# tan9zj/xnrs

Measured on AMD Instinct MI355X. Metric: impressions/sec (encode+score) on MIND-shaped batches, higher is better.
Workload: dtype f32; 1 GPU; NRMS full user+news encode + 5-candidate dot scoring (BASELINE configs[2]; token shape of config/mind_small_NRMS.yml); batch_impressions_per_gpu=512, history=50, candidates=5, d_backbone=768, n_heads=16, emb_dim=256, parallelism=impressions sharded by user over 1 GPU(s), no data-path collective

## Files before the change

include/xnrs_hip.h:

```cpp
#ifndef XNRS_HIP_H
#define XNRS_HIP_H

#include <stddef.h>
#include <stdint.h>

#ifdef __cplusplus
extern "C" {
#endif

#define XNRS_ABI_VERSION 6

#define XNRS_OK 0
#define XNRS_EINVAL (-1)
#define XNRS_EHEADS (-2)
#define XNRS_EWORKSPACE (-3)
#define XNRS_EUNSUPPORTED (-4)

#define XNRS_ACT_NONE 0
#define XNRS_ACT_RELU 1
#define XNRS_ACT_TANH 2

#define XNRS_POOL_ADDITIVE 0
#define XNRS_POOL_MEAN 1

// ... 185 lines not shown
                          uint64_t seed, const uint64_t *seed_dev, void *stream);

int32_t xnrs_gather_rows_bf16(const uint16_t *table, const int32_t *ids, float *out, int64_t n, int64_t row_elems,
                              void *stream);
int32_t xnrs_dropout_rows_bf16(const uint16_t *table, const int32_t *ids, float *out, int64_t n, int64_t row_elems,
                               float p, uint64_t seed, const uint64_t *seed_dev, void *stream);

int32_t xnrs_assemble_train_batch(const int64_t *sess, int64_t B, const int64_t *hist_off, const int32_t *hist_val,
                                  const int64_t *pos_off, const int32_t *pos_val, const int64_t *neg_off,
                                  const int32_t *neg_val, int32_t l_hist, int32_t n_neg, int32_t pad_row, uint64_t seed,
                                  int32_t *hist_rows, int32_t *cand_rows, void *stream);
int32_t xnrs_assemble_eval_batch(const int64_t *sess, int64_t B, const int64_t *hist_off, const int32_t *hist_val,
                                 const int64_t *pos_off, const int32_t *pos_val, const int64_t *neg_off,
                                 const int32_t *neg_val, int32_t l_hist, int32_t pad_row, const int64_t *cand_off,
                                 int32_t *hist_rows, int32_t *cand_rows, int32_t *cand_sess, float *targets, void *stream);
int32_t xnrs_score_csr(const float *vecs, const int32_t *cand_rows, const int32_t *cand_sess, const float *u, float *r,
                       int64_t n_cand, int32_t E, int32_t relu, void *stream);
int32_t xnrs_rank_metrics(const float *scores, const float *targets, const int64_t *cand_off, float *out, int64_t B,
                          void *stream);

size_t xnrs_infonce_saved_bytes(int64_t B, int32_t E);
int32_t xnrs_infonce_fwd(const float *emb, const int64_t *labels, int64_t B, int32_t E, float temperature, float *loss,
                         void *saved, size_t saved_bytes, void *stream);
int32_t xnrs_infonce_bwd(const int64_t *labels, int64_t B, int32_t E, float temperature, const void *saved,
                         size_t saved_bytes, const float *gout, float *demb, void *stream);

#define XNRS_PROFILE_STAGES 10
int32_t xnrs_profile_enable(uint32_t stage_mask);
int32_t xnrs_profile_read(double *ms, int64_t *launches, double *flops);

int32_t xnrs_qkv_launch_count(int32_t reset);
int32_t xnrs_qkv_one_launch_map(int64_t block, int64_t live_tiles, int64_t live_rows, int32_t kv_row_tiles,
                                int32_t kv_col_tiles, int64_t q_rows, int32_t q_tile_rows, int32_t q_col_tiles,
                                int32_t *section, int32_t *index);

int32_t xnrs_train_fold_enabled(void);

#define XNRS_STATUS_NONBINARY_MASK 1
#define XNRS_STATUS_ROW_RANGE 2
#define XNRS_STATUS_QUERY_RANGE 4
int32_t xnrs_set_status_word(int32_t *device_word);
const char *xnrs_status_string(int32_t word);

#define XNRS_GEMM_F32 0
#define XNRS_GEMM_BF16X3 1
#define XNRS_GEMM_BF16X2 2
int32_t xnrs_set_gemm_mode(int32_t mode);
int32_t xnrs_get_gemm_mode(void);

int32_t xnrs_reload_knobs(void);

size_t xnrs_bilinear_scoring_saved_bytes(int64_t B, int32_t E, int32_t normalize);
int32_t xnrs_bilinear_scoring_fwd(const float *u, const float *c, const float *w, const float *bias, float *s, int64_t B,
                                  int32_t N, int32_t E, int32_t normalize, void *saved, size_t saved_bytes, void *stream);
size_t xnrs_bilinear_scoring_bwd_workspace_bytes(int64_t B, int32_t E, int32_t normalize);
int32_t xnrs_bilinear_scoring_bwd(const float *u, const float *c, const float *w, const void *saved, size_t saved_bytes,
                                  const float *ds, float *du, float *dc, float *dw, float *dbias, int64_t B, int32_t N,
                                  int32_t E, int32_t normalize, void *ws, size_t ws_bytes, void *stream);
size_t xnrs_mlp_scoring_saved_bytes(int64_t B, int32_t N, int32_t H);
int32_t xnrs_mlp_scoring_fwd(const float *u, const float *c, const float *w1, const float *b1, const float *w2,
                             const float *b2, float *s, int64_t B, int32_t N, int32_t E, int32_t H, void *saved,
                             size_t saved_bytes, void *stream);
size_t xnrs_mlp_scoring_bwd_workspace_bytes(int64_t B, int32_t N, int32_t H);
int32_t xnrs_mlp_scoring_bwd(const float *u, const float *c, const float *w1, const float *w2, const void *saved,
                             size_t saved_bytes, const float *ds, float *du, float *dc, float *dw1, float *db1, float *dw2,
                             float *db2, int64_t B, int32_t N, int32_t E, int32_t H, void *ws, size_t ws_bytes,
// ... 93 lines not shown
```

xnrs_amd/csrc/api.hip:

```cpp
#include <mutex>
#include <vector>

#include "host.h"

using namespace xnrs;

namespace xnrs {
uint32_t g_prof_mask = 0;
}
namespace {
std::vector<ProfRec> g_prof;
std::mutex g_prof_mu;
constexpr size_t PROF_MAX = 1 << 16;
}

bool xnrs::prof_begin(ProfRec* r, hipStream_t stream) {
  if (hipEventCreate(&r->beg) != hipSuccess || hipEventCreate(&r->end) != hipSuccess) return false;
  (void)hipEventRecord(r->beg, stream);
  return true;
}

void xnrs::prof_end(const ProfRec& r, hipStream_t stream) {
  (void)hipEventRecord(r.end, stream);
  std::lock_guard<std::mutex> lk(g_prof_mu);
// ... 56 lines not shown
  const int prev = xnrs::gemm_mode();
  xnrs::set_gemm_mode(mode);
  return prev;
}

int32_t xnrs_get_gemm_mode(void) { return xnrs::gemm_mode(); }

int32_t xnrs_train_fold_enabled(void) { return fold_wanted(knobs().fold_train) ? 1 : 0; }

int32_t xnrs_reload_knobs(void) {
  xnrs::reload_knobs();
  return XNRS_OK;
}

int32_t xnrs_qkv_launch_count(int32_t reset) {
  const int64_t n = xnrs::qkv_launches_read(reset != 0);
  return n > 0x7fffffffLL ? 0x7fffffff : (int32_t)n;
}

int32_t xnrs_qkv_one_launch_map(int64_t block, int64_t live_tiles, int64_t live_rows, int32_t kv_row_tiles, int32_t kv_col_tiles,
                                int64_t q_rows, int32_t q_tile_rows, int32_t q_col_tiles, int32_t* section, int32_t* index) {
  if (kv_row_tiles < 0 || kv_col_tiles < 1 || q_rows < 0 || q_tile_rows < 1 || q_col_tiles < 1) return XNRS_EINVAL;
  const int64_t grid = xnrs::qkv_one_launch_grid(kv_row_tiles, kv_col_tiles, q_rows, q_tile_rows, q_col_tiles);
  if (grid > 0x7fffffffLL) return XNRS_EINVAL;
  if (section && index) {
    const xnrs::QkvOneLaunchWork w =
        xnrs::qkv_one_launch_map(block, live_tiles, live_rows, kv_row_tiles, kv_col_tiles, q_rows, q_tile_rows, q_col_tiles);
    *section = w.section;
    *index = w.index;
  }
  return (int32_t)grid;
}

int32_t xnrs_profile_enable(uint32_t stage_mask) {
  std::lock_guard<std::mutex> lk(g_prof_mu);
  for (auto& r : g_prof) {
    (void)hipEventDestroy(r.beg);
    (void)hipEventDestroy(r.end);
  }
  g_prof.clear();
  g_prof_mask = stage_mask;
  return XNRS_OK;
}

int32_t xnrs_profile_read(double* ms, int64_t* launches, double* flops) {
  if (!ms || !launches || !flops) return XNRS_EINVAL;
  for (int i = 0; i < XNRS_PROFILE_STAGES; ++i) {
    ms[i] = 0.0;
    launches[i] = 0;
    flops[i] = 0.0;
  }
  int32_t rc = XNRS_OK;
  std::lock_guard<std::mutex> lk(g_prof_mu);
  for (auto& r : g_prof) {
    float t = 0.f;
    hipError_t e = hipEventSynchronize(r.end);
    if (e == hipSuccess) e = hipEventElapsedTime(&t, r.beg, r.end);
    if (e != hipSuccess) rc = (int32_t)e;
    else {
      ms[r.stage] += t;
      launches[r.stage] += 1;
      flops[r.stage] += r.flops;
    }
    (void)hipEventDestroy(r.beg);
    (void)hipEventDestroy(r.end);
  }
// ... 6 lines not shown
```

xnrs_amd/csrc/encoder_fwd.hip:

```cpp
#include <vector>

#include "host.h"

using namespace xnrs;

namespace xnrs {

Plan make_plan(int64_t n_seq, int L, int D, int A, int E, bool att, bool additive, bool head, bool pooled, int64_t chunk,
               bool train, int n_heads, bool widen) {
  Plan p{};
  if (train) chunk = n_seq > 0 ? n_seq : 1;
  if (chunk <= 0) chunk = 65536 / L;
  if (chunk > n_seq) chunk = n_seq;
  if (chunk < 1) chunk = 1;
  p.chunk = chunk;
  const size_t rows = (size_t)chunk * L;
  Carver c;
  p.off_qkv = c.take_if(att, rows * 3 * (size_t)D * F32);
  p.off_o = c.take_if(att, rows * (size_t)D * F32);
  p.off_y = c.take_if(att && pooled, rows * (size_t)D * F32);
  p.off_t = c.take_if(pooled && additive, rows * (size_t)A * F32);
  p.off_p = c.take_if(pooled && head, (size_t)n_seq * D * F32);
  p.off_h = c.take_if(pooled && head, (size_t)n_seq * E * F32);
  p.off_stats = c.take_if(train && att, (size_t)chunk * n_heads * L * 2 * F32);
// ... 369 lines not shown
    probe.mask = m;
    probe.skip_dead = 1;
    lt_qkv = mha_core_skips_dead(probe);
  }
  const bool lt_fc1 = lt && additive && rowdot;
  const int64_t lt_cap = live_tiles_cap(p.chunk, L, LIVE_TILE_BM);
  const int64_t* lt_n = at<int64_t>(w, p.off_lt_n);
  const int32_t* lt_tiles = at<int32_t>(w, p.off_lt_tiles);
  const bool lr = lt && knobs().gemm_live_rows && p.off_lr_cnt != 0 && L <= 64 && n_seq * (int64_t)L <= 0x7fffffffLL &&
                  n_seq * (int64_t)L >= knobs().gemm_live_rows_min_rows;
  const bool lr_qkv = lr && lt_qkv && !direct, lr_fc1 = lr && lt_fc1;
  const int32_t *lr_loc = at<int32_t>(w, p.off_lr_loc), *lr_src = at<int32_t>(w, p.off_lr_src);
  const int64_t* lr_cnt = at<int64_t>(w, p.off_lr_cnt);
  constexpr float LR_FILL = 0.3f;
  if (lr_qkv || lr_fc1)
    XNRS_TRY(launch_dense_row_lists(m, ids, n_seq, p.chunk, L, LIVE_TILE_BM, at<int32_t>(w, p.off_lr_loc), at<int32_t>(w, p.off_lr_src),
                                    at<int64_t>(w, p.off_lr_cnt), at<uint8_t>(w, p.off_lt_alive), at<int64_t>(w, p.off_lt_n),
                                    at<int32_t>(w, p.off_lt_tiles), stream));
  else if (lt_qkv || lt_fc1)
    XNRS_TRY(launch_live_tiles(m, ids, n_seq, p.chunk, L, LIVE_TILE_BM, at<uint8_t>(w, p.off_lt_alive), at<int64_t>(w, p.off_lt_n),
                               at<int32_t>(w, p.off_lt_tiles), stream));
  std::vector<int64_t> lt_host, lr_host;
  if ((lt_qkv && prof_on(0)) || (lt_fc1 && prof_on(3))) {
    lt_host.resize((size_t)((n_seq + p.chunk - 1) / p.chunk));
    if (hipStreamSynchronize(stream) != hipSuccess ||
        hipMemcpy(lt_host.data(), lt_n, lt_host.size() * sizeof(int64_t), hipMemcpyDeviceToHost) != hipSuccess)
      lt_host.clear();
    if (lr_qkv || lr_fc1) {
      lr_host.resize(3 * lt_host.size());
      if (lt_host.empty() || hipMemcpy(lr_host.data(), lr_cnt, lr_host.size() * sizeof(int64_t), hipMemcpyDeviceToHost) != hipSuccess)
        lr_host.clear();
    }
  }
  for (int64_t c0 = 0; !fused && !afused && c0 < n_seq; c0 += p.chunk) {
    const int64_t nc = (n_seq - c0 < p.chunk) ? (n_seq - c0) : p.chunk;
    const int64_t rows = nc * L;
    const int64_t* ltn = lt_n + c0 / p.chunk;
    const int32_t* ltl = lt_tiles + (c0 / p.chunk) * lt_cap;
    const double lt_rows = (double)LIVE_TILE_BM *
                           (double)(lt_host.empty() ? (rows + LIVE_TILE_BM - 1) / LIVE_TILE_BM : lt_host[(size_t)(c0 / p.chunk)]);
    const int32_t* lrl = lr_loc + (c0 / p.chunk) * p.chunk * L;
    const int32_t* lrs = lr_src + (c0 / p.chunk) * p.chunk * L;
    const int64_t* lrn = lr_cnt + 3 * (c0 / p.chunk);
    const double lr_rows = lr_host.empty() ? (double)rows : (double)lr_host[(size_t)(3 * (c0 / p.chunk))];
    const int32_t* cids = ids ? ids + c0 : nullptr;
    const float* cx = ids ? x : x + c0 * (int64_t)L * D;
    const float* cm = m ? (ids ? m : m + c0 * (int64_t)L) : nullptr;
    const int32_t* xids = cids;
    if (x16) {
      cx = direct ? nullptr : x32;
      xids = direct ? cids : nullptr;
      if (!direct) XNRS_TRY(widen_pass(c0, nc, false));
    }

    const float* seq = cx;
    const int32_t* seq_ids = xids;
    if (att) {
      const int64_t ld3 = 3 * (int64_t)D;
      if (qkv_given) {
      } else if (live) {
        const double nl = (double)prof_count(0, cnt, 0, n_live, stream), nkv = (double)prof_count(0, cnt, 1, n_kv, stream);
        ProfScope ps(0, 2.0 * (kvl ? nkv : rows) * 2.0 * D * D + 2.0 * nl * (double)D * D, stream);
        GemmArgs g = qkv_projection(cx, {xids, L}, att, 1, qkv + D, ld3, rows, D, pqkv);
        if (kvl) {
          XNRS_TRY(launch_zero_dead_qkv(qkv, cm, cids, nc, L, D, stream));
          g.gather_ids = kvx;
          g.gather_S = 1;
          g.c_scatter = 1;
          g.c_scatter_ids = kv_rows;
          g.M = n_kv;
          g.m_dev = cnt ? cnt + 1 : nullptr;
          g.m_fill_hint = 0.6f;
          if (n_kv > 0) XNRS_TRY(launch_gemm_f32(g, stream));
        } else {
          XNRS_TRY(launch_gemm_f32(g, stream));
          XNRS_TRY(launch_zero_cols(qkv, ld3, D, rows, stream));
        }
        if (n_live > 0) {
          GemmArgs q = gemm_linear(cx, {lvx, 1}, D, att->wq, att->bq, qkv, ld3, n_live, D, D, XNRS_ACT_NONE, pqkv[0]);
          q.c_scatter = 1;
          q.c_scatter_ids = live_rows;
          q.m_dev = cnt;
          q.m_fill_hint = 0.4f;
          XNRS_TRY(launch_gemm_f32(q, stream));
        }
      } else if (lr_qkv) {
        ProfScope ps(0, 2.0 * lt_rows * 2.0 * D * D + 2.0 * lr_rows * (double)D * D, stream);
        GemmArgs g = qkv_projection(cx, {xids, L}, att, 1, qkv + D, ld3, rows, D, pqkv);
        g.live_n = ltn;
        g.live_tiles = ltl;
        GemmArgs q = gemm_linear(cx, {xids ? lrs : lrl, 1}, D, att->wq, att->bq, qkv, ld3, rows, D, D);
        q.c_scatter = 1;
        q.c_scatter_ids = lrl;
        q.m_dev = lrn;
        q.m_fill_hint = LR_FILL;
        if (gemm_qkv_one_launch_ok(g, q)) {
          XNRS_TRY(launch_gemm_qkv_one(g, q, stream));
          qkv_launches_add(1);
        } else {
          XNRS_TRY(launch_gemm_f32(g, stream));
          XNRS_TRY(launch_gemm_f32(q, stream));
          qkv_launches_add(2);
        }
      } else {
        GemmArgs g = qkv_projection(cx, {xids, L}, att, 0, qkv, ld3, rows, D, pqkv);
        if (lt_qkv) {
          g.live_n = ltn;
          g.live_tiles = ltl;
        }
        ProfScope ps(0, 2.0 * (lt_qkv ? lt_rows : (double)rows) * 3.0 * D * D, stream);
        if (direct) XNRS_TRY(launch_gemm_a16(g, x16, stream));
        else XNRS_TRY(launch_gemm_f32(g, stream));
      }

      MhaCoreArgs ma = mha_core_args(qkv + D, ld3, att, o, nc, L, D);
      ma.q = qkv;
      ma.mask = cm;
      ma.mask_gather_ids = cids;
      ma.dropout_p = att->dropout_p;
      ma.seed = att->seed + (uint64_t)c0 * (uint64_t)att->n_heads * 0x9E3779B97F4A7C15ull;
      ma.seed_dev = att->seed_dev;
      ma.stats = stats;
      ma.skip_dead = (live || (pooled && cm && knobs().mha_skip_masked)) ? 1 : 0;
      if (lt_qkv && !mha_core_skips_dead(ma)) return XNRS_EUNSUPPORTED;
      {
        ProfScope ps(1, 4.0 * rows * (double)L * D, stream);
        XNRS_TRY(launch_mha_core(ma, stream));
      }

      float* dst = pooled ? yb : y + c0 * (int64_t)L * D;
      if (fold) {
        dst = o;
      } else if (live) {
        ProfScope ps(2, 2.0 * (double)prof_count(2, cnt, 0, n_live, stream) * (double)D * D, stream);
        XNRS_TRY(hipMemsetAsync(dst, 0, (size_t)rows * D * sizeof(float), stream));
// ... 3 lines not shown
          og.m_dev = cnt;
          og.m_fill_hint = 0.4f;
          XNRS_TRY(launch_gemm_f32(og, stream));
        }
      } else {
        ProfScope ps(2, 2.0 * rows * (double)D * D, stream);
        XNRS_TRY(launch_gemm_f32(gemm_linear(o, {}, D, att->wo, att->bo, dst, D, rows, D, D, XNRS_ACT_NONE, po), stream));
      }
      seq = dst;
      seq_ids = nullptr;
    }
    if (!pooled) continue;

    float* pooled_dst = (head ? pb : y) + c0 * (int64_t)D;
    float* hm_dst = hm ? hm + c0 : nullptr;
    if (additive) {
      if (live) {
        ProfScope ps(3, 2.0 * (double)prof_count(3, cnt, 0, n_live, stream) * (double)D * A, stream);
        XNRS_TRY(hipMemsetAsync(t, 0, (size_t)rows * A * sizeof(float), stream));
        if (n_live > 0) {
          GemmArgs fg = fc1_product(seq, {att ? live_rows : lvx, 1}, fc1, t, n_live, D, A, false, pool, p1);
          fg.c_scatter = 1;
          fg.c_scatter_ids = live_rows;
          fg.m_dev = cnt;
          fg.m_fill_hint = 0.4f;
          XNRS_TRY(launch_gemm_f32(fg, stream));
        }
      } else if (lr_fc1) {
        GemmArgs fg = fc1_product(seq, {seq_ids ? lrs : lrl, 1}, fc1, t, rows, D, A, true, pool, p1);
        fg.c_scatter = 1;
        fg.c_scatter_ids = lrl;
        fg.m_dev = lrn;
        fg.m_fill_hint = LR_FILL;
        ProfScope ps(3, 2.0 * lr_rows * (double)D * A, stream);
        XNRS_TRY(launch_gemm_f32(fg, stream));
      } else {
        GemmArgs fg = fc1_product(seq, {seq_ids, L}, fc1, t, rows, D, A, rowdot, pool, p1);
        if (lt_fc1) {
          fg.live_n = ltn;
          fg.live_tiles = ltl;
        }
        ProfScope ps(3, 2.0 * (lt_fc1 ? lt_rows : (double)rows) * (double)D * A, stream);
        XNRS_TRY(launch_gemm_f32(fg, stream));
      }
      AdditivePoolArgs pa = additive_pool_args(t, rowdot, pool, seq, nc, L, D, A);
      pa.skip_dead = lt_fc1 ? 1 : 0;
      pa.skip_masked = lr_fc1 ? 1 : 0;
      pa.mask = cm;
      pa.mask_gather_ids = cids;
      pa.x_gather_ids = seq_ids;
      pa.y = fold ? pob + c0 * (int64_t)D : pooled_dst;
      pa.asum_out = fold ? asum + c0 : nullptr;
      pa.a_out = a_save ? a_save : (a_out ? a_out + c0 * (int64_t)L : nullptr);
      pa.hm_out = cm ? hm_dst : nullptr;
      {
        ProfScope ps(4, 2.0 * rows * (double)(A + D), stream);
        XNRS_TRY(launch_additive_pool(pa, stream));
      }
      if (a_save && a_out)
        XNRS_TRY(hipMemcpyAsync(a_out, a_save, (size_t)rows * sizeof(float), hipMemcpyDeviceToDevice, stream));
    } else {
      MeanPoolArgs mp{};
      mp.x = seq;
      mp.ldx = D;
      mp.mask = cm;
      mp.mask_gather_ids = cids;
      mp.x_gather_ids = seq_ids;
      mp.y = pooled_dst;
      mp.hm_out = hm_dst;
      mp.n_seq = nc;
      mp.N = L;
      mp.D = D;
      {
        ProfScope ps(4, 2.0 * rows * (double)D, stream);
        XNRS_TRY(launch_mean_pool(mp, stream));
      }
    }
  }
  return pooled_tail(fold, pob, asum, att, pooled ? head : nullptr, pb, hb, y, n_seq, D, E, po, train, stream);
}

namespace {

struct UnpadPlan {
  size_t off_kv, off_q, off_o, off_y, off_t, off_p, off_h;
  FoldRegions fold;
  size_t total;
};
UnpadPlan make_unpad_plan(int64_t n_news, int64_t n_valid, int S, int D, int A, int E, bool att, bool head) {
  UnpadPlan p{};
  Carver c;
  const size_t nv = (size_t)(n_valid > 0 ? n_valid : 1);
  p.off_kv = c.take_if(att, (size_t)n_news * S * 2 * D * F32);
  p.off_q = c.take_if(att, nv * D * F32);
  p.off_o = c.take_if(att, nv * D * F32);
  p.off_y = c.take_if(att, nv * D * F32);
  p.off_t = c.take(nv * A * F32);
  p.off_p = c.take_if(head, (size_t)n_news * D * F32);
  p.off_h = c.take_if(head, (size_t)n_news * E * F32);
  p.fold = carve_fold(c, att, n_news, D, A);
  p.total = c.total();
  return p;
}

struct CompactPlan {
  int64_t chunk;
  size_t off_kv, off_q, off_o, off_t, off_roff, off_live, off_kvs, off_kvb, off_cnt, off_p, off_h;
  FoldRegions fold;
  size_t total;
};
CompactPlan make_compact_plan(int64_t n_news, int S, int D, int A, int E, bool att, bool head, int64_t chunk) {
// ... 339 lines not shown
```

xnrs_amd/csrc/gemm_f32.hip:

```cpp
#include <atomic>
#include <cstdlib>
#include <type_traits>

#include "kernels.h"

namespace xnrs {

constexpr int KALIGN = 32;

__device__ __attribute__((aligned(16))) float g_zero_line[4] = {0.f, 0.f, 0.f, 0.f};

typedef unsigned u32x4 __attribute__((ext_vector_type(4)));
constexpr unsigned BUF_OOB = 0x40000000u;

template <int TM, int TN, bool A_COL, bool B_KN, bool VEC, int PIPE, int BK, bool BUF = false, int MINW = 2, bool GATH = false,
          int KG = 2, bool RDOT = false, bool MDEV = false, bool LIVE = false>
__global__ __launch_bounds__(256, MINW) void gemm_f32_kernel(const GemmArgs a, int m_tiles, int n_tiles_seg, int gn) {
#define XNRS_GEMM_BID blockIdx.x
#define XNRS_GEMM_NWG gridDim.x
#define XNRS_GEMM_LDS_TILES(A, B)                            \
  __shared__ __attribute__((aligned(16))) float A[NBUF][A_SZ]; \
  __shared__ __attribute__((aligned(16))) float B[NBUF][B_SZ];
#include "gemm_f32_body.h"
#undef XNRS_GEMM_BID
// ... 9 lines not shown
template <int TM, int TN, bool A_COL, bool B_KN, bool VEC, int PIPE, int BK, bool BUF = false, int MINW = 2, bool GATH = false,
          int KG = 2, bool RDOT = false, bool MDEV = false, bool LIVE = false>
__device__ __forceinline__ void gemm_f32_body(const GemmArgs& a, int m_tiles, const int n_tiles_seg, const int gn, const int bid_in,
                                              const int nwg_in, float* As0, float* Bs0) {
  static_assert(!A_COL && !B_KN, "forward layout (the LDS tile sizes of gemm_f32_lds_floats)");
#define XNRS_GEMM_BID bid_in
#define XNRS_GEMM_NWG nwg_in
#define XNRS_GEMM_LDS_TILES(A, B)                                                                                   \
  static_assert(NBUF * A_SZ == gemm_f32_lds_floats<TM, BK>() && NBUF * B_SZ == gemm_f32_lds_floats<TN, BK>(), "LDS"); \
  float(*const A)[A_SZ] = reinterpret_cast<float(*)[A_SZ]>(As0);                                                    \
  float(*const B)[B_SZ] = reinterpret_cast<float(*)[B_SZ]>(Bs0);
#include "gemm_f32_body.h"
#undef XNRS_GEMM_BID
#undef XNRS_GEMM_NWG
#undef XNRS_GEMM_LDS_TILES
}

__global__ __launch_bounds__(256, 4) void gemm_qkv_one_launch_kernel(const GemmArgs kv, const GemmArgs q, int kv_m_tiles,
                                                                     int kv_n_tiles_seg, int kv_gn, int q_m_tiles, int q_n_tiles,
                                                                     int q_gn) {
  __shared__ __attribute__((aligned(16))) float As[gemm_f32_lds_floats<2, 16>()];
  __shared__ __attribute__((aligned(16))) float Bs[gemm_f32_lds_floats<2, 16>()];
  static_assert(sizeof(As) + sizeof(Bs) <= 32768, "four workgroups per CU");
  const int64_t ln = __builtin_amdgcn_readfirstlane((int)load_dev_scalar(kv.live_n));
  const int64_t md0 = load_dev_scalar(q.m_dev);
  const int64_t md = ((int64_t)__builtin_amdgcn_readfirstlane((int)(md0 >> 32)) << 32) | (uint32_t)__builtin_amdgcn_readfirstlane((int)md0);
  const QkvOneLaunchWork w = qkv_one_launch_map((int64_t)blockIdx.x, ln, md, kv_m_tiles, kv_n_tiles_seg * kv.nseg, q.M, 128, q_n_tiles);
  if (w.section < 0) return;
  if (w.section == 0)
    gemm_f32_body<2, 2, false, false, true, 5, 16, true, 4, false, 2, false, false, true>(kv, kv_m_tiles, kv_n_tiles_seg, kv_gn, w.index, 0,
                                                                                        As, Bs);
  else
    gemm_f32_body<2, 1, false, false, true, 5, 16, true, 4, true, 2, false, true, false>(q, q_m_tiles, q_n_tiles, q_gn, w.index, 0, As, Bs);
}

__global__ __launch_bounds__(256) void transpose_kernel(const float* W, float* Wt, int rows, int cols) {
  __shared__ float tile[32][33];
  const int tx = threadIdx.x & 31, ty = threadIdx.x >> 5;
  const int c0 = blockIdx.x * 32, r0 = blockIdx.y * 32;
#pragma unroll
  for (int i = 0; i < 4; ++i) {
    const int r = r0 + ty + 8 * i, c = c0 + tx;
    if (r < rows && c < cols) tile[ty + 8 * i][tx] = W[(int64_t)r * cols + c];
  }
  __syncthreads();
#pragma unroll
  for (int i = 0; i < 4; ++i) {
    const int c = c0 + ty + 8 * i, r = r0 + tx;
    if (r < rows && c < cols) Wt[(int64_t)c * rows + r] = tile[tx][ty + 8 * i];
  }
}

__global__ __launch_bounds__(256) void zero_cols_kernel(float* p, int64_t ld, int w4, int64_t n4) {
  const int64_t i = (int64_t)blockIdx.x * 256 + threadIdx.x;
  if (i >= n4) return;
  const int64_t r = i / w4;
  const int c = (int)(i - r * w4);
  __builtin_nontemporal_store(f32x4{0.f, 0.f, 0.f, 0.f}, reinterpret_cast<f32x4*>(p + r * ld) + c);
}

hipError_t launch_zero_cols(float* p, int64_t ld, int width, int64_t rows, hipStream_t stream) {
  if (rows <= 0 || width <= 0) return hipSuccess;
  if (width % 4 != 0 || ld % 4 != 0 || (reinterpret_cast<uintptr_t>(p) & 15) != 0)
    return hipMemset2DAsync(p, (size_t)ld * sizeof(float), 0, (size_t)width * sizeof(float), (size_t)rows, stream);
  const int64_t n4 = rows * (width / 4);
  hipLaunchKernelGGL(zero_cols_kernel, dim3((unsigned)((n4 + 255) / 256)), dim3(256), 0, stream, p, ld, width / 4, n4);
// ... 206 lines not shown
  return (int)ns;
}

static Knobs read_knobs() {
  Knobs k;
  auto num = [](const char* name, long long dflt) {
    const char* e = getenv(name);
    return (e && *e) ? atoll(e) : dflt;
  };
  k.gemm_pipe = (int)num("XNRS_GEMM_PIPE", 6);
  k.gemm_bk = num("XNRS_GEMM_BK", 32) == 16 ? 16 : 32;
  k.gemm_buf = num("XNRS_GEMM_BUF", 1) != 0;
  k.gemm_group = num("XNRS_GEMM_GROUP", -1);
  k.gemm_tile = (int)num("XNRS_GEMM_TILE", -1);
  k.split_min_tiles = num("XNRS_GEMM_SPLIT_MIN_TILES", 512);
  k.mha_lds = (int)num("XNRS_MHA_LDS", -1);
  k.mha_headwave = num("XNRS_MHA_HEADWAVE", 1) != 0;
  k.mha_pair = num("XNRS_MHA_PAIR", 1) != 0;
  k.mha_bwd_fused = num("XNRS_MHA_BWD_FUSED", 1) != 0;
  k.gemm_dw = (int)num("XNRS_GEMM_DW", 2);
  k.gemm_dw_tile = (int)num("XNRS_GEMM_DW_TILE", 256);
  k.fold_out = (int)num("XNRS_FOLD_OUT", 1);
  k.fc1_rowdot = num("XNRS_FC1_ROWDOT", 1) != 0;
  k.fold_train = (int)num("XNRS_FOLD_TRAIN", 1);
  k.news_fused = (int)num("XNRS_NEWS_FUSED", 1);
  k.news_fused_npw = (int)num("XNRS_NEWS_FUSED_NPW", 0);
  k.fast_tanh = num("XNRS_FAST_TANH", 1) != 0;
  k.additive_fused = (int)num("XNRS_ADDITIVE_FUSED", 1);
  k.af_fbuf = num("XNRS_AF_FBUF", 1) == 2 ? 2 : 1;
  k.mha_skip_masked = num("XNRS_MHA_SKIP_MASKED", 1) != 0;
  {
    k.gemm_qkv_one_launch = num("XNRS_GEMM_QKV_ONE_LAUNCH", 1) != 0;
  }
  k.gemm_live_tiles = num("XNRS_GEMM_LIVE_TILES", 1) != 0;
  k.gemm_live_tiles_min_rows = num("XNRS_GEMM_LIVE_TILES_MIN_ROWS", 16384);
  k.gemm_live_rows = num("XNRS_GEMM_LIVE_ROWS", 1) != 0;
  k.gemm_live_rows_min_rows = num("XNRS_GEMM_LIVE_ROWS_MIN_ROWS", 16384);
  k.bwd_side_stream = num("XNRS_BWD_SIDE_STREAM", 1) != 0;
  k.bwd_side_min_rows = num("XNRS_BWD_SIDE_MIN_ROWS", 0);
  k.gru_layout = num("XNRS_GRU_LAYOUT", 0) == 1 ? 1 : 0;
  k.gemm_a16 = num("XNRS_GEMM_A16", 1) != 0;
  const long long m = num("XNRS_GEMM_MODE", 0);
  k.gemm_mode_init = (m >= 0 && m <= 2) ? (int)m : 0;
  return k;
}
static Knobs g_knobs = read_knobs();
static std::atomic<int> g_gemm_mode{g_knobs.gemm_mode_init};
const Knobs& knobs() { return g_knobs; }
void reload_knobs() { g_knobs = read_knobs(); }
int gemm_mode() { return g_gemm_mode.load(std::memory_order_relaxed); }
void set_gemm_mode(int mode) { g_gemm_mode.store((mode >= 0 && mode <= 2) ? mode : 0, std::memory_order_relaxed); }

hipError_t launch_gemm_f32(const GemmArgs& a_in, hipStream_t stream, int* nsplit_used) {
  GemmArgs a = a_in;
  if (a.M <= 0 || a.Nseg <= 0) return hipSuccess;
  if (a.act == 2 && knobs().fast_tanh) a.act = ACT_TANH_FAST;
  if (a.K >= (1ll << 31)) return hipErrorInvalidValue;
  auto al16 = [](const void* p) { return (reinterpret_cast<uintptr_t>(p) & 15) == 0; };
  bool vec = (a.lda % 4 == 0) && (a.ldw % 4 == 0) && al16(a.A);
  vec = vec && (a.a_col ? (a.M % 4 == 0) : (a.K % 4 == 0));
  vec = vec && (a.b_kn ? (a.Nseg % 4 == 0) : (a.K % 4 == 0));
  for (int s = 0; s < a.nseg; ++s) vec = vec && al16(a.W[s]);

  int nsplit = 1;
  if (a.slabs && a.nsplit > 1) {
    nsplit = a.nsplit;
// ... 69 lines not shown
  if (!knobs().gemm_buf || (int64_t)a.Nseg * a.ldw * 4 > (int64_t)BUF_OOB) return false;
  *gath = a.gather_ids || a.M * a.lda * 4 > (int64_t)BUF_OOB;
  return true;
}

bool gemm_qkv_one_launch_ok(const GemmArgs& kv, const GemmArgs& q) {
  if (!knobs().gemm_qkv_one_launch || gemm_mode() != 0 || knobs().gemm_tile >= 0) return false;
  bool kv_gath = false, q_gath = false;
  if (!qkv_section_ok(kv, &kv_gath) || !qkv_section_ok(q, &q_gath)) return false;
  if (kv_gath || !kv.live_tiles || !kv.live_n || kv.m_dev || kv.c_scatter) return false;
  if (!q_gath || !q.gather_ids || q.gather_S != 1 || !q.c_scatter || !q.m_dev || q.live_tiles || q.nseg != 1) return false;
  const int64_t grid = qkv_one_launch_grid((int)((kv.M + 127) / 128), (kv.Nseg + 127) / 128 * kv.nseg, q.M, 128, (q.Nseg + 63) / 64);
  return (kv.M + 127) / 128 <= 0x7fffffffLL && grid <= 0x7fffffffLL;
}

hipError_t launch_gemm_qkv_one(const GemmArgs& kv_in, const GemmArgs& q_in, hipStream_t stream) {
  if (!gemm_qkv_one_launch_ok(kv_in, q_in)) return hipErrorInvalidValue;
  GemmArgs kv = kv_in, q = q_in;
  for (GemmArgs* a : {&kv, &q}) {
    if (a->act == 2 && knobs().fast_tanh) a->act = ACT_TANH_FAST;
    a->k_per_split = a->K;
    a->nt_store = (!a->accumulate && !a->c_scatter && a->M * a->ldc * 4 >= (64ll << 20)) ? 1 : 0;
  }
  const int kv_m_tiles = (int)((kv.M + 127) / 128), kv_n_tiles_seg = (kv.Nseg + 127) / 128;
  const int q_m_tiles = (int)((q.M + 127) / 128), q_n_tiles = (q.Nseg + 63) / 64;
  const int kv_gn = gemm_group_tiles(kv_n_tiles_seg * kv.nseg, 128, kv.K, false);
  const int q_gn = gemm_group_tiles(q_n_tiles, 64, q.K, false);
  const dim3 g((unsigned)qkv_one_launch_grid(kv_m_tiles, kv_n_tiles_seg * kv.nseg, q.M, 128, q_n_tiles));
  hipLaunchKernelGGL(gemm_qkv_one_launch_kernel, g, dim3(256), 0, stream, kv, q, kv_m_tiles, kv_n_tiles_seg, kv_gn, q_m_tiles, q_n_tiles,
                     q_gn);
  return hipGetLastError();
}

}
```

xnrs_amd/csrc/kernels.h:

```cpp
#pragma once
#include <hip/hip_runtime.h>
#include <stdint.h>

namespace xnrs {

typedef float f32x4 __attribute__((ext_vector_type(4)));
typedef float f32x16 __attribute__((ext_vector_type(16)));

struct Knobs {
  int gemm_pipe = 6;
  int gemm_bk = 32;
  int gemm_buf = 1;
  long long gemm_group = -1;
  int gemm_tile = -1;
  long long split_min_tiles = 512;
  bool fc1_rowdot = true;
  int fold_train = 1;
  int fold_out = 1;
  int gemm_dw = 2;
  int gemm_dw_tile = 256;
  int mha_lds = -1;
  bool mha_pair = true;
  int mha_headwave = 1;
  int mha_bwd_fused = 1;
  int news_fused = 1;
  int news_fused_npw = 0;
  int gemm_mode_init = 0;
  bool fast_tanh = true;
  int additive_fused = 1;
  int af_fbuf = 1;
  bool bwd_side_stream = true;
  long long bwd_side_min_rows = 0;
  bool gemm_live_tiles = true;
  long long gemm_live_tiles_min_rows = 16384;
  bool gemm_live_rows = true;
  long long gemm_live_rows_min_rows = 16384;
  bool gemm_qkv_one_launch = true;
  bool mha_skip_masked = true;
  bool gemm_a16 = true;
  int gru_layout = 0;
};
const Knobs& knobs();
void reload_knobs();

__device__ __forceinline__ int64_t load_dev_scalar(const int64_t* p) { return *p; }

struct GemmArgs {
  const float* A;
  int32_t a_col;
  const int32_t* gather_ids;
  int32_t gather_S;
  int32_t c_scatter;
  const int32_t* c_scatter_ids;
  int64_t lda;
  const float* W[3];
  const float* bias[3];
  int32_t b_kn;
  const int32_t* b_gather_ids;
  int32_t b_gather_S;
  int32_t nseg;
  int32_t Nseg;
  int64_t ldw;
  float* C;
  int64_t ldc;
  int64_t M;
  int64_t K;
  int32_t act;
  const float* aux;
  int64_t ldaux;
  int32_t aux_mode;
// ... 18 lines not shown
  const int32_t* live_tiles;
  float* slabs;
  int32_t nsplit;
  int64_t k_per_split;
  int64_t slab_stride;
};
hipError_t launch_zero_cols(float* p, int64_t ld, int width, int64_t rows, hipStream_t stream);
hipError_t launch_zero_dead_qkv(float* qkv, const float* mask, const int32_t* ids, int64_t n_seq, int L, int D, hipStream_t stream);
hipError_t launch_transpose(const float* W, float* Wt, int rows, int cols, hipStream_t stream);
int gemm_pick_splits(int64_t M, int64_t N, int64_t K, bool dw_kernel = false);
int gemm_group_tiles(int n_tiles, int bn, int64_t K, bool plain);
size_t gemm_splitk_workspace_bytes(int64_t M, int64_t N, int64_t K);
hipError_t launch_gemm_f32(const GemmArgs& a, hipStream_t stream, int* nsplit_used = nullptr);
struct QkvOneLaunchWork {
  int section;
  int index;
};
__host__ __device__ inline QkvOneLaunchWork qkv_one_launch_map(int64_t block, int64_t live_n, int64_t m_dev, int kv_m_tiles,
                                                               int kv_n_tiles, int64_t q_rows, int q_bm, int q_n_tiles) {
  const int64_t lt = live_n < kv_m_tiles ? (live_n > 0 ? live_n : 0) : kv_m_tiles;
  const int64_t kv_wgs = lt * kv_n_tiles, kv_pad = (kv_wgs + 7) & ~(int64_t)7;
  if (block < kv_pad) return block >= 0 && block < kv_wgs ? QkvOneLaunchWork{0, (int)block} : QkvOneLaunchWork{-1, 0};
  const int64_t rows = m_dev < q_rows ? (m_dev > 0 ? m_dev : 0) : q_rows;
  const int64_t q_wgs = ((rows + q_bm - 1) / q_bm) * q_n_tiles;
  return block - kv_pad < q_wgs ? QkvOneLaunchWork{1, (int)(block - kv_pad)} : QkvOneLaunchWork{-1, 0};
}
inline int64_t qkv_one_launch_grid(int kv_m_tiles, int kv_n_tiles, int64_t q_rows, int q_bm, int q_n_tiles) {
  return (((int64_t)kv_m_tiles * kv_n_tiles + 7) & ~(int64_t)7) + ((q_rows + q_bm - 1) / q_bm) * q_n_tiles;
}
bool gemm_qkv_one_launch_ok(const GemmArgs& kv, const GemmArgs& q);
hipError_t launch_gemm_qkv_one(const GemmArgs& kv, const GemmArgs& q, hipStream_t stream);
void qkv_launches_add(int n);
int64_t qkv_launches_read(bool reset);
bool gemm_dw_eligible(const GemmArgs& a);
bool gemm_dw_big_tile(const GemmArgs& a);
hipError_t launch_gemm_dw(const GemmArgs& a, int nsplit, hipStream_t stream);
hipError_t launch_gemm_split(const GemmArgs& a, int npl, hipStream_t stream);
inline int64_t split_plane_ld(int64_t K) { return (K + 15) / 16 * 16; }
inline size_t split_planes_bytes(int64_t N, int64_t K) { return (size_t)3 * (size_t)N * (size_t)split_plane_ld(K) * 2; }
hipError_t launch_split_weights(const float* W, int64_t N, int64_t K, unsigned short* planes, hipStream_t stream);
bool gemm_a16_ok(const GemmArgs& a, const unsigned short* A16, bool check_size = true);
hipError_t launch_gemm_a16(const GemmArgs& a, const unsigned short* A16, hipStream_t stream);
int gemm_mode();
void set_gemm_mode(int mode);

struct MhaCoreArgs {
  const float* q;
  const float* k;
  const float* v;
  int64_t ld;
  int64_t seq_stride;
  int64_t head_stride;
  const float* mask;
  const int32_t* mask_gather_ids;
  float* out;
  int64_t ldo;
  int64_t n_seq;
  int32_t S, n_heads, d_k;
  int32_t scaled;
  float dropout_p;
  uint64_t seed;
  const uint64_t* seed_dev;
  float* stats;
  const int64_t* q_off;
  int64_t ldq;
  const int32_t* kv_block;
// ... 351 lines not shown
```

Before: 21330 impressions/s.

## Defer chunk fc1 GEMM into the next chunk's fused QKV launch tail

When the encoder runs in chunks with live-row QKV and fc1 projections, each chunk's additive-attention fc1 GEMM is held back. It is then issued as a third section of the next chunk's single QKV launch, and the additive pool runs afterwards. The aim is to save one launch per chunk and to fill the otherwise idle tail workgroups of the QKV grid with fc1 tiles. The cost is more complex scheduling, a pending-state drain at the end, and fc1 tiles fixed at 64x64 inside the shared kernel.

```diff
diff --git a/include/xnrs_hip.h b/include/xnrs_hip.h
--- a/include/xnrs_hip.h
+++ b/include/xnrs_hip.h
@@ -241,6 +241,12 @@
 int32_t xnrs_qkv_launch_count(int32_t reset);
 int32_t xnrs_qkv_one_launch_map(int64_t block, int64_t live_tiles, int64_t live_rows, int32_t kv_row_tiles,
                                 int32_t kv_col_tiles, int64_t q_rows, int32_t q_tile_rows, int32_t q_col_tiles,
+                                int32_t *section, int32_t *index);
+
+int32_t xnrs_fc1_in_tail_count(int32_t reset);
+int32_t xnrs_qkv_fc1_launch_map(int64_t block, int64_t live_tiles, int64_t live_rows, int64_t fc1_live_rows,
+                                int32_t kv_row_tiles, int32_t kv_col_tiles, int64_t q_rows, int32_t q_tile_rows,
+                                int32_t q_col_tiles, int64_t fc1_rows, int32_t fc1_tile_rows, int32_t fc1_col_tiles,
                                 int32_t *section, int32_t *index);
 
 int32_t xnrs_train_fold_enabled(void);
diff --git a/xnrs_amd/csrc/api.hip b/xnrs_amd/csrc/api.hip
--- a/xnrs_amd/csrc/api.hip
+++ b/xnrs_amd/csrc/api.hip
@@ -112,6 +112,29 @@
   return (int32_t)grid;
 }
 
+int32_t xnrs_fc1_in_tail_count(int32_t reset) {
+  const int64_t n = xnrs::fc1_in_tail_read(reset != 0);
+  return n > 0x7fffffffLL ? 0x7fffffff : (int32_t)n;
+}
+
+int32_t xnrs_qkv_fc1_launch_map(int64_t block, int64_t live_tiles, int64_t live_rows, int64_t fc1_live_rows, int32_t kv_row_tiles,
+                                int32_t kv_col_tiles, int64_t q_rows, int32_t q_tile_rows, int32_t q_col_tiles, int64_t fc1_rows,
+                                int32_t fc1_tile_rows, int32_t fc1_col_tiles, int32_t* section, int32_t* index) {
+  if (kv_row_tiles < 0 || kv_col_tiles < 1 || q_rows < 0 || q_tile_rows < 1 || q_col_tiles < 1 || fc1_rows < 0 || fc1_tile_rows < 1 ||
+      fc1_col_tiles < 1)
+    return XNRS_EINVAL;
+  const int64_t grid =
+      xnrs::qkv_fc1_launch_grid(kv_row_tiles, kv_col_tiles, q_rows, q_tile_rows, q_col_tiles, fc1_rows, fc1_tile_rows, fc1_col_tiles);
+  if (grid > 0x7fffffffLL) return XNRS_EINVAL;
+  if (section && index) {
+    const xnrs::QkvOneLaunchWork w = xnrs::qkv_fc1_launch_map(block, live_tiles, live_rows, fc1_live_rows, kv_row_tiles, kv_col_tiles, q_rows,
+                                                              q_tile_rows, q_col_tiles, fc1_rows, fc1_tile_rows, fc1_col_tiles);
+    *section = w.section;
+    *index = w.index;
+  }
+  return (int32_t)grid;
+}
+
 int32_t xnrs_profile_enable(uint32_t stage_mask) {
   std::lock_guard<std::mutex> lk(g_prof_mu);
   for (auto& r : g_prof) {
diff --git a/xnrs_amd/csrc/encoder_fwd.hip b/xnrs_amd/csrc/encoder_fwd.hip
--- a/xnrs_amd/csrc/encoder_fwd.hip
+++ b/xnrs_amd/csrc/encoder_fwd.hip
@@ -425,6 +425,39 @@
         lr_host.clear();
     }
   }
+  const bool tail = lr_qkv && lr_fc1 && fold && pooled && !ids && !x16 && !qkv_given && !live && knobs().gemm_fc1_in_tail &&
+                    !prof_on(3);
+  auto pool_pass = [&](int64_t c0, int64_t nc, const float* cm, const int32_t* cids, const float* seq, const int32_t* seq_ids) -> int32_t {
+    AdditivePoolArgs pa = additive_pool_args(t, rowdot, pool, seq, nc, L, D, A);
+    pa.skip_dead = lt_fc1 ? 1 : 0;
+    pa.skip_masked = lr_fc1 ? 1 : 0;
+    pa.mask = cm;
+    pa.mask_gather_ids = cids;
+    pa.x_gather_ids = seq_ids;
+    pa.y = fold ? pob + c0 * (int64_t)D : (head ? pb : y) + c0 * (int64_t)D;
+    pa.asum_out = fold ? asum + c0 : nullptr;
+    pa.a_out = a_save ? a_save : (a_out ? a_out + c0 * (int64_t)L : nullptr);
+    pa.hm_out = (cm && hm) ? hm + c0 : nullptr;
+    {
+      ProfScope ps(4, 2.0 * (double)(nc * L) * (double)(A + D), stream);
+      XNRS_TRY(launch_additive_pool(pa, stream));
+    }
+    if (a_save && a_out)
+      XNRS_TRY(hipMemcpyAsync(a_out, a_save, (size_t)(nc * L) * sizeof(float), hipMemcpyDeviceToDevice, stream));
+    return XNRS_OK;
+  };
+  struct {
+    bool on = false;
+    GemmArgs fg;
+    int64_t c0 = 0, nc = 0;
+    const float* cm = nullptr;
+  } pend;
+  auto drain = [&]() -> int32_t {
+    if (!pend.on) return XNRS_OK;
+    pend.on = false;
+    XNRS_TRY(launch_gemm_f32(pend.fg, stream));
+    return pool_pass(pend.c0, pend.nc, pend.cm, nullptr, o, nullptr);
+  };
   for (int64_t c0 = 0; !fused && !afused && c0 < n_seq; c0 += p.chunk) {
     const int64_t nc = (n_seq - c0 < p.chunk) ? (n_seq - c0) : p.chunk;
     const int64_t rows = nc * L;
@@ -478,7 +511,6 @@
           XNRS_TRY(launch_gemm_f32(q, stream));
         }
       } else if (lr_qkv) {
-        ProfScope ps(0, 2.0 * lt_rows * 2.0 * D * D + 2.0 * lr_rows * (double)D * D, stream);
         GemmArgs g = qkv_projection(cx, {xids, L}, att, 1, qkv + D, ld3, rows, D, pqkv);
         g.live_n = ltn;
         g.live_tiles = ltl;
@@ -487,13 +519,27 @@
         q.c_scatter_ids = lrl;
         q.m_dev = lrn;
         q.m_fill_hint = LR_FILL;
-        if (gemm_qkv_one_launch_ok(g, q)) {
-          XNRS_TRY(launch_gemm_qkv_one(g, q, stream));
-          qkv_launches_add(1);
-        } else {
-          XNRS_TRY(launch_gemm_f32(g, stream));
-          XNRS_TRY(launch_gemm_f32(q, stream));
-          qkv_launches_add(2);
+        const bool one = gemm_qkv_one_launch_ok(g, q);
+        const bool merged = tail && one && (!pend.on || gemm_fc1_in_tail_ok(pend.fg));
+        if (!merged) XNRS_TRY_RC(drain());
+        {
+          ProfScope ps(0, 2.0 * lt_rows * 2.0 * D * D + 2.0 * lr_rows * (double)D * D, stream);
+          if (merged) {
+            XNRS_TRY(launch_gemm_qkv_fc1(g, q, pend.on ? &pend.fg : nullptr, stream));
+            qkv_launches_add(1);
+            if (pend.on) fc1_in_tail_add(1);
+          } else if (one) {
+            XNRS_TRY(launch_gemm_qkv_one(g, q, stream));
+            qkv_launches_add(1);
+          } else {
+            XNRS_TRY(launch_gemm_f32(g, stream));
+            XNRS_TRY(launch_gemm_f32(q, stream));
+            qkv_launches_add(2);
+          }
+        }
+        if (pend.on) {
+          pend.on = false;
+          XNRS_TRY_RC(pool_pass(pend.c0, pend.nc, pend.cm, nullptr, o, nullptr));
         }
       } else {
         GemmArgs g = qkv_projection(cx, {xids, L}, att, 0, qkv, ld3, rows, D, pqkv);
@@ -563,6 +609,14 @@
         fg.c_scatter_ids = lrl;
         fg.m_dev = lrn;
         fg.m_fill_hint = LR_FILL;
+        if (tail) {
+          pend.on = true;
+          pend.fg = fg;
+          pend.c0 = c0;
+          pend.nc = nc;
+          pend.cm = cm;
+          continue;
+        }
         ProfScope ps(3, 2.0 * lr_rows * (double)D * A, stream);
         XNRS_TRY(launch_gemm_f32(fg, stream));
       } else {
@@ -574,22 +628,7 @@
         ProfScope ps(3, 2.0 * (lt_fc1 ? lt_rows : (double)rows) * (double)D * A, stream);
         XNRS_TRY(launch_gemm_f32(fg, stream));
       }
-      AdditivePoolArgs pa = additive_pool_args(t, rowdot, pool, seq, nc, L, D, A);
-      pa.skip_dead = lt_fc1 ? 1 : 0;
-      pa.skip_masked = lr_fc1 ? 1 : 0;
-      pa.mask = cm;
-      pa.mask_gather_ids = cids;
-      pa.x_gather_ids = seq_ids;
-      pa.y = fold ? pob + c0 * (int64_t)D : pooled_dst;
-      pa.asum_out = fold ? asum + c0 : nullptr;
-      pa.a_out = a_save ? a_save : (a_out ? a_out + c0 * (int64_t)L : nullptr);
-      pa.hm_out = cm ? hm_dst : nullptr;
-      {
-        ProfScope ps(4, 2.0 * rows * (double)(A + D), stream);
-        XNRS_TRY(launch_additive_pool(pa, stream));
-      }
-      if (a_save && a_out)
-        XNRS_TRY(hipMemcpyAsync(a_out, a_save, (size_t)rows * sizeof(float), hipMemcpyDeviceToDevice, stream));
+      XNRS_TRY_RC(pool_pass(c0, nc, cm, cids, seq, seq_ids));
     } else {
       MeanPoolArgs mp{};
       mp.x = seq;
@@ -608,6 +647,7 @@
       }
     }
   }
+  XNRS_TRY_RC(drain());
   return pooled_tail(fold, pob, asum, att, pooled ? head : nullptr, pb, hb, y, n_seq, D, E, po, train, stream);
 }
 
diff --git a/xnrs_amd/csrc/gemm_f32.hip b/xnrs_amd/csrc/gemm_f32.hip
--- a/xnrs_amd/csrc/gemm_f32.hip
+++ b/xnrs_amd/csrc/gemm_f32.hip
@@ -65,6 +65,33 @@
                                                                                         As, Bs);
   else
     gemm_f32_body<2, 1, false, false, true, 5, 16, true, 4, true, 2, false, true, false>(q, q_m_tiles, q_n_tiles, q_gn, w.index, 0, As, Bs);
+}
+
+template <int FTM, int FTN>
+__global__ __launch_bounds__(256, 4) void gemm_qkv_fc1_launch_kernel(const GemmArgs kv, const GemmArgs q, const GemmArgs f, int kv_m_tiles,
+                                                                     int kv_n_tiles_seg, int kv_gn, int q_m_tiles, int q_n_tiles, int q_gn,
+                                                                     int f_m_tiles, int f_n_tiles, int f_gn) {
+  __shared__ __attribute__((aligned(16))) float As[gemm_f32_lds_floats<2, 16>()];
+  __shared__ __attribute__((aligned(16))) float Bs[gemm_f32_lds_floats<2, 16>()];
+  static_assert(sizeof(As) + sizeof(Bs) <= 32768, "four workgroups per CU");
+  static_assert(FTM >= 1 && FTM <= 2 && FTN >= 1 && FTN <= 2, "the third section's tiles fit the arrays of the first");
+  auto dev64 = [](const int64_t* p) {
+    const int64_t v = load_dev_scalar(p);
+    return ((int64_t)__builtin_amdgcn_readfirstlane((int)(v >> 32)) << 32) | (uint32_t)__builtin_amdgcn_readfirstlane((int)v);
+  };
+  const int64_t ln = __builtin_amdgcn_readfirstlane((int)load_dev_scalar(kv.live_n));
+  const int64_t md = dev64(q.m_dev);
+  const int64_t fd = f.M > 0 ? dev64(f.m_dev) : 0;
+  const QkvOneLaunchWork w = qkv_fc1_launch_map((int64_t)blockIdx.x, ln, md, fd, kv_m_tiles, kv_n_tiles_seg * kv.nseg, q.M, 128, q_n_tiles,
+                                                f.M, 64 * FTM, f_n_tiles);
+  if (w.section < 0) return;
+  if (w.section == 0)
+    gemm_f32_body<2, 2, false, false, true, 5, 16, true, 4, false, 2, false, false, true>(kv, kv_m_tiles, kv_n_tiles_seg, kv_gn, w.index, 0,
+                                                                                        As, Bs);
+  else if (w.section == 1)
+    gemm_f32_body<2, 1, false, false, true, 5, 16, true, 4, true, 2, false, true, false>(q, q_m_tiles, q_n_tiles, q_gn, w.index, 0, As, Bs);
+  else
+    gemm_f32_body<FTM, FTN, false, false, true, 5, 16, true, 4, true, 2, true, true, false>(f, f_m_tiles, f_n_tiles, f_gn, w.index, 0, As, Bs);
 }
 
 __global__ __launch_bounds__(256) void transpose_kernel(const float* W, float* Wt, int rows, int cols) {
@@ -337,6 +364,7 @@
   {
     k.gemm_qkv_one_launch = num("XNRS_GEMM_QKV_ONE_LAUNCH", 1) != 0;
   }
+  k.gemm_fc1_in_tail = num("XNRS_GEMM_FC1_IN_TAIL", 1) != 0;
   k.gemm_live_tiles = num("XNRS_GEMM_LIVE_TILES", 1) != 0;
   k.gemm_live_tiles_min_rows = num("XNRS_GEMM_LIVE_TILES_MIN_ROWS", 16384);
   k.gemm_live_rows = num("XNRS_GEMM_LIVE_ROWS", 1) != 0;
@@ -472,4 +500,44 @@
   return hipGetLastError();
 }
 
-}
+static std::atomic<int64_t> g_fc1_in_tail{0};
+void fc1_in_tail_add(int n) { g_fc1_in_tail.fetch_add(n, std::memory_order_relaxed); }
+int64_t fc1_in_tail_read(bool reset) {
+  return reset ? g_fc1_in_tail.exchange(0, std::memory_order_relaxed) : g_fc1_in_tail.load(std::memory_order_relaxed);
+}
+
+bool gemm_fc1_in_tail_ok(const GemmArgs& f) {
+  auto al16 = [](const void* p) { return (reinterpret_cast<uintptr_t>(p) & 15) == 0; };
+  if (!knobs().gemm_fc1_in_tail || gemm_mode() != 0 || knobs().gemm_tile >= 0 || !knobs().gemm_buf) return false;
+  if (f.a_col || f.b_kn || f.M <= 0 || f.Nseg <= 0 || f.nseg != 1 || f.K < 4 || f.K >= (1ll << 31) || f.K % 4 != 0) return false;
+  if (f.lda % 4 != 0 || f.ldw % 4 != 0 || !al16(f.A) || !al16(f.W[0]) || (int64_t)f.Nseg * f.ldw * 4 > (int64_t)BUF_OOB) return false;
+  if ((f.slabs && f.nsplit > 1) || f.rowscale || f.colsum || f.k_dev || f.C2 || f.live_tiles || f.accumulate || f.aux_mode) return false;
+  if (!f.rowdot_out || !f.rowdot_w || (f.act != 2 && f.act != ACT_TANH_FAST)) return false;
+  if (!f.gather_ids || f.gather_S != 1 || !f.c_scatter || !f.m_dev) return false;
+  return (f.M + FC1_TAIL_BM - 1) / FC1_TAIL_BM * ((f.Nseg + FC1_TAIL_BN - 1) / FC1_TAIL_BN) <= 0x3fffffffLL;
+}
+
+hipError_t launch_gemm_qkv_fc1(const GemmArgs& kv_in, const GemmArgs& q_in, const GemmArgs* f_in, hipStream_t stream) {
+  if (!gemm_qkv_one_launch_ok(kv_in, q_in) || (f_in && !gemm_fc1_in_tail_ok(*f_in))) return hipErrorInvalidValue;
+  GemmArgs kv = kv_in, q = q_in, f{};
+  if (f_in) f = *f_in;
+  for (GemmArgs* a : {&kv, &q, &f}) {
+    if (a->act == 2 && knobs().fast_tanh) a->act = ACT_TANH_FAST;
+    a->k_per_split = a->K > 0 ? a->K : 1;
+    a->nt_store = (!a->accumulate && !a->c_scatter && a->M * a->ldc * 4 >= (64ll << 20)) ? 1 : 0;
+  }
+  constexpr int FTM = FC1_TAIL_BM / 64, FTN = FC1_TAIL_BN / 64;
+  const int kv_m_tiles = (int)((kv.M + 127) / 128), kv_n_tiles_seg = (kv.Nseg + 127) / 128;
+  const int q_m_tiles = (int)((q.M + 127) / 128), q_n_tiles = (q.Nseg + 63) / 64;
+  const int f_m_tiles = (int)((f.M + FC1_TAIL_BM - 1) / FC1_TAIL_BM), f_n_tiles = f_in ? (f.Nseg + FC1_TAIL_BN - 1) / FC1_TAIL_BN : 1;
+  const int kv_gn = gemm_group_tiles(kv_n_tiles_seg * kv.nseg, 128, kv.K, false);
+  const int q_gn = gemm_group_tiles(q_n_tiles, 64, q.K, false);
+  const int f_gn = gemm_group_tiles(f_n_tiles, FC1_TAIL_BN, f.K, false);
+  const int64_t grid = qkv_fc1_launch_grid(kv_m_tiles, kv_n_tiles_seg * kv.nseg, q.M, 128, q_n_tiles, f.M, FC1_TAIL_BM, f_n_tiles);
+  if (grid <= 0 || grid > 0x7fffffffLL) return hipErrorInvalidValue;
+  hipLaunchKernelGGL((gemm_qkv_fc1_launch_kernel<FTM, FTN>), dim3((unsigned)grid), dim3(256), 0, stream, kv, q, f, kv_m_tiles, kv_n_tiles_seg,
+                     kv_gn, q_m_tiles, q_n_tiles, q_gn, f_m_tiles, f_n_tiles, f_gn);
+  return hipGetLastError();
+}
+
+}
diff --git a/xnrs_amd/csrc/kernels.h b/xnrs_amd/csrc/kernels.h
--- a/xnrs_amd/csrc/kernels.h
+++ b/xnrs_amd/csrc/kernels.h
@@ -36,6 +36,7 @@
   bool gemm_live_rows = true;
   long long gemm_live_rows_min_rows = 16384;
   bool gemm_qkv_one_launch = true;
+  bool gemm_fc1_in_tail = true;
   bool mha_skip_masked = true;
   bool gemm_a16 = true;
   int gru_layout = 0;
@@ -120,6 +121,29 @@
 hipError_t launch_gemm_qkv_one(const GemmArgs& kv, const GemmArgs& q, hipStream_t stream);
 void qkv_launches_add(int n);
 int64_t qkv_launches_read(bool reset);
+__host__ __device__ inline QkvOneLaunchWork qkv_fc1_launch_map(int64_t block, int64_t live_n, int64_t m_dev, int64_t f_dev, int kv_m_tiles,
+                                                               int kv_n_tiles, int64_t q_rows, int q_bm, int q_n_tiles, int64_t f_rows,
+                                                               int f_bm, int f_n_tiles) {
+  const QkvOneLaunchWork w = qkv_one_launch_map(block, live_n, m_dev, kv_m_tiles, kv_n_tiles, q_rows, q_bm, q_n_tiles);
+  if (w.section >= 0) return w;
+  const int64_t lt = live_n < kv_m_tiles ? (live_n > 0 ? live_n : 0) : kv_m_tiles;
+  const int64_t rows = m_dev < q_rows ? (m_dev > 0 ? m_dev : 0) : q_rows;
+  const int64_t q_end = ((lt * kv_n_tiles + 7) & ~(int64_t)7) + ((rows + q_bm - 1) / q_bm) * q_n_tiles;
+  const int64_t f0 = (q_end + 7) & ~(int64_t)7;
+  const int64_t fr = f_dev < f_rows ? (f_dev > 0 ? f_dev : 0) : f_rows;
+  const int64_t f_wgs = ((fr + f_bm - 1) / f_bm) * f_n_tiles;
+  return block >= f0 && block - f0 < f_wgs ? QkvOneLaunchWork{2, (int)(block - f0)} : QkvOneLaunchWork{-1, 0};
+}
+inline int64_t qkv_fc1_launch_grid(int kv_m_tiles, int kv_n_tiles, int64_t q_rows, int q_bm, int q_n_tiles, int64_t f_rows, int f_bm,
+                                   int f_n_tiles) {
+  return ((qkv_one_launch_grid(kv_m_tiles, kv_n_tiles, q_rows, q_bm, q_n_tiles) + 7) & ~(int64_t)7) +
+         ((f_rows + f_bm - 1) / f_bm) * f_n_tiles;
+}
+constexpr int FC1_TAIL_BM = 64, FC1_TAIL_BN = 64;
+bool gemm_fc1_in_tail_ok(const GemmArgs& f);
+hipError_t launch_gemm_qkv_fc1(const GemmArgs& kv, const GemmArgs& q, const GemmArgs* f, hipStream_t stream);
+void fc1_in_tail_add(int n);
+int64_t fc1_in_tail_read(bool reset);
 bool gemm_dw_eligible(const GemmArgs& a);
 bool gemm_dw_big_tile(const GemmArgs& a);
 hipError_t launch_gemm_dw(const GemmArgs& a, int nsplit, hipStream_t stream);
```

After: 21690 impressions/s (median of 6 runs). 1.02x the previous value.
